# PKU-MARL/HARL

Hardware: AMD Instinct MI355X
Metric: transitions/sec through HAPPO update (MPE spread, 3 agents) (higher is better)
Workload: dtype f32; 1 GPU; MPE simple_spread_v2 3-agent HAPPO update: compute_returns + train(), T=200, n_rollout_threads=4096/GPU (4096 global, weak scaling), obs18/share54/Box5, MLP[128, 128], ppo_epoch=5, critic_epoch=5; episode_length=200, n_rollout_threads_per_gpu=4096, n_rollout_threads_global=4096, n_agents=3, parallelism=dp1, collective=none, world_size=1, ranks_seen=1

## Files before the change

### harl_amd/csrc/bwd_fused.h

```cpp
#pragma once

__device__ __forceinline__ unsigned split_stage1(float f0, float f1, float &r0, float &r1) {
  const unsigned b0 = __float_as_uint(f0), b1 = __float_as_uint(f1);
  r0 = f0 - __uint_as_float(b0 & 0xffff0000u);
  r1 = f1 - __uint_as_float(b1 & 0xffff0000u);
  return __builtin_amdgcn_perm(b1, b0, 0x07060302u);
}
__device__ __forceinline__ void split_stage2(float r0, float r1, unsigned &p2, unsigned &p3) {
  const unsigned c0 = __float_as_uint(r0), c1 = __float_as_uint(r1);
  p2 = __builtin_amdgcn_perm(c1, c0, 0x07060302u);
  const float q0 = r0 - __uint_as_float(c0 & 0xffff0000u), q1 = r1 - __uint_as_float(c1 & 0xffff0000u);
  p3 = __builtin_amdgcn_perm(__float_as_uint(q1), __float_as_uint(q0), 0x07060302u);
}

template <int I, int N, typename F>
__device__ __forceinline__ void static_for(F &&f) {
  if constexpr (I < N) {
    f(std::integral_constant<int, I>{});
    static_for<I + 1, N>(f);
  }
}

constexpr int BDW_H = 128, BDW_MT = 4, BDW_NJ = 8, BDW_NR = 64, BDW_KPF = 32;
constexpr int BDW_SQ = (128 / 16) * 128 + 8, BDW_IMG = 8 * BDW_SQ;
constexpr int BDW_BUF = 3 * BDW_IMG;
constexpr size_t bdw_lds_bytes() { return split_image_bytes(128, 128) + (size_t)2 * BDW_BUF; }

template <int N>
__device__ __forceinline__ void zero_acc(f32x16 (&a)[N], float *db = nullptr) {
#pragma unroll
  for (int t = 0; t < N; ++t) {
    if (db) db[t] = 0.f;
#pragma unroll
    for (int r = 0; r < 16; ++r) a[t][r] = 0.f;
  }
}

struct GradRounds {
  static constexpr int H = BDW_H;
  const float *const dz, *const xprev;
  const long n_slabs;
  unsigned char *const Bb;
  const int lane, wave, i, h;
  const Ident ident;
  f32x16 acc2[4];
  float db2;
  f32x4 prA[4], prB[4];
  u32x2_t spB[4][3];
  u32x4 ya[3][2];
  f32x16 tc[3];
  u32x4 At[3][2], AtN[3][2];
  float rr0, rr1;
  float vnext;
  const int frag_lane;

  __device__ __forceinline__ GradRounds(const float *dz_, const float *xprev_, long n_slabs_, unsigned char *Bb_, int lane_,
                                        int wave_, const Ident &ident_)
      : dz(dz_), xprev(xprev_), n_slabs(n_slabs_), Bb(Bb_), lane(lane_), wave(wave_), i(lane_ & 31), h(lane_ >> 5),
        ident(ident_), db2(0.f), rr0(0.f), rr1(0.f), vnext(1.f),
        frag_lane(((lane_ >> 4) & 1) * 128 + ((lane_ & 15) >> 2) * 32 + (lane_ & 3) * 8) {}

  __device__ __forceinline__ void d_load(long ds) {
#pragma unroll
    for (int u = 0; u < 4; ++u) {
      prA[u] = (reinterpret_cast<const f32x4 *>(dz + ds * (long)(H * SLAB)) + lane)[(4 * wave + u) * WAVE];
      prB[u] = (reinterpret_cast<const f32x4 *>(xprev + ds * (long)(H * SLAB)) + lane)[(4 * wave + u) * WAVE];
    }
  }
  __device__ __forceinline__ void d_load_next(long ds, long fallback) { d_load(ds < n_slabs ? ds : fallback); }
  __device__ __forceinline__ void a_chunk(int k) {
    const int pi = k >> 1, j = pi >> 2, c = pi & 3, u = pi >> 1, e = 2 * (pi & 1);
    if ((k & 1) == 0) {
      ya[0][j][c] = split_stage1(prA[u][e], prA[u][e + 1], rr0, rr1);
    } else {
      unsigned p2, p3;
      split_stage2(rr0, rr1, p2, p3);
      ya[1][j][c] = p2;
      ya[2][j][c] = p3;
    }
  }
  __device__ __forceinline__ void b_chunk(int k) {
    const int u = k >> 2, c2 = (k >> 1) & 1;
    if ((k & 1) == 0) {
      spB[u][0][c2] = split_stage1(prB[u][2 * c2], prB[u][2 * c2 + 1], rr0, rr1);
    } else {
      unsigned p2, p3;
      split_stage2(rr0, rr1, p2, p3);
      spB[u][1][c2] = p2;
      spB[u][2][c2] = p3;
    }
  }
  __device__ __forceinline__ void t_mfma(int k) {
    const f32x16 zero = {0.f, 0.f, 0.f, 0.f, 0.f, 0.f, 0.f, 0.f, 0.f, 0.f, 0.f, 0.f, 0.f, 0.f, 0.f, 0.f};
    const int t = k % 3;
    if (k < 3) tc[t] = mfma_bf16(ya[t][0], ident.j0, zero);
    else tc[t] = mfma_bf16(ya[t][1], ident.j1, tc[t]);
  }
  __device__ __forceinline__ void p_chunk(int k) {
    if (k < 3) {
      pack_transposed(tc[k], AtN[k][0], AtN[k][1]);
    } else {
      f32x2 a = {0.f, 0.f};
#pragma unroll
      for (int r = 0; r < 8; ++r) a += f32x2{tc[k - 3][2 * r], tc[k - 3][2 * r + 1]};
      db2 += vnext * (a[0] + a[1]);
    }
  }
  __device__ __forceinline__ void b_store(int buf) {
#pragma unroll
    for (int u = 0; u < 4; ++u) {
      const int q = 4 * wave + u;
      unsigned char *d = Bb + buf * BDW_BUF + (i >> 2) * BDW_SQ + (2 * (q >> 2) + ((q & 3) >> 1)) * 128 + (i & 3) * 32 +
                         (8 * (q & 1) + 4 * h) * 2;
#pragma unroll
      for (int term = 0; term < 3; ++term) *reinterpret_cast<u32x2_t *>(d + term * BDW_IMG) = spB[u][term];
    }
  }
  __device__ __forceinline__ void read_frag(int buf, int ks, int tile, u32x4 (&f)[3]) {
#pragma unroll
    for (int term = 0; term < 3; ++term) {
      const unsigned char *fp = Bb + buf * BDW_BUF + term * BDW_IMG + (4 * ks + h) * BDW_SQ + 2 * tile * 128 + frag_lane;
      const u32x2_t lo = tr_read(fp), hi = tr_read(fp + 2 * BDW_SQ);
      f[term] = u32x4{lo[0], lo[1], hi[0], hi[1]};
    }
  }
  __device__ __forceinline__ void a_advance() {
#pragma unroll
    for (int t = 0; t < 3; ++t) {
      At[t][0] = AtN[t][0];
      At[t][1] = AtN[t][1];
    }
  }

  __device__ __forceinline__ void prologue(long base0) {
    d_load(base0);
#pragma unroll
    for (int k = 0; k < 16; ++k) a_chunk(k);
#pragma unroll
    for (int k = 0; k < 6; ++k) t_mfma(k);
#pragma unroll
    for (int k = 0; k < 16; ++k) b_chunk(k);
#pragma unroll
    for (int k = 0; k < 6; ++k) p_chunk(k);
    a_advance();
    b_store(0);
  }

  template <int r, bool FILL, class Sched, class Extra, class Phase>
  __device__ __forceinline__ void round(long base, long sr_stride, Extra &&extra, Phase &&phase) {
    __syncthreads();
    phase(std::integral_constant<int, 5>{});
    const long ds1 = r < 3 ? base + r + 1 : base + sr_stride;
    const long ds2 = r < 2 ? base + r + 2 : base + sr_stride;
    vnext = uniform_f(ds1 < n_slabs ? 1.f : 0.f);
    constexpr int TSLOT = r == 0 ? 31 : 15;
    auto slot = [&](auto sc) {
      constexpr int s_ = decltype(sc)::value;
      if constexpr (r == 0) {
        if constexpr (s_ >= 16 && s_ < 32) a_chunk(s_ - 16);
        else if constexpr (s_ >= 32 && s_ < 42) b_chunk(s_ - 32 + 6);
        else if constexpr (s_ >= 42) p_chunk(s_ - 42);
        if constexpr (s_ == Sched::LOAD_R0) d_load_next(ds2, base);
      } else {
        if constexpr (s_ < 16) a_chunk(s_);
        else if constexpr (s_ < 26) b_chunk(s_ - 16 + 6);
        else if constexpr (s_ < 32) p_chunk(s_ - 26);
        else extra(std::integral_constant<int, r>{}, sc);
        if constexpr (s_ == Sched::LOAD_RN && r < 3) d_load_next(ds2, base);
      }
      if constexpr (s_ == TSLOT) {
        static_for<0, 6>([&](auto kc) {
          constexpr int k = decltype(kc)::value;
          __builtin_amdgcn_sched_barrier(0);
          t_mfma(k);
          b_chunk(k);
        });
      }
    };
    u32x4 bv[2][3];
    read_frag(r & 1, 0, 0, bv[0]);
    if constexpr (!FILL) static_for<0, 48>(slot);
    static_for<0, 8>([&](auto nc) {
      constexpr int n = decltype(nc)::value, ks = n >> 2, b = n & 3;
      if constexpr (n + 1 < 8) read_frag(r & 1, (n + 1) >> 2, (n + 1) & 3, bv[(n + 1) & 1]);
      __builtin_amdgcn_sched_barrier(0);
      constexpr int AT[6] = {2, 0, 1, 1, 0, 0}, BT[6] = {0, 2, 1, 0, 1, 0};
      static_for<0, 6>([&](auto kc) {
        constexpr int k6 = decltype(kc)::value;
        acc2[b] = mfma_bf16(At[AT[k6]][ks], bv[n & 1][BT[k6]], acc2[b]);
        if constexpr (FILL) slot(std::integral_constant<int, 6 * n + k6>{});
        __builtin_amdgcn_sched_barrier(0);
      });
    });
    phase(std::integral_constant<int, 6>{});
    b_store((r + 1) & 1);
    a_advance();
    phase(std::integral_constant<int, 7>{});
  }

  template <bool FILL, class Sched, class Extra, class Phase>
  __device__ __forceinline__ void rounds(long base, long sr_stride, Extra &&extra, Phase &&phase) {
    static_for<0, 4>([&](auto rc) {
      constexpr int r = decltype(rc)::value;
      if (base + r < n_slabs) round<r, FILL, Sched>(base, sr_stride, extra, phase);
    });
  }

  __device__ __forceinline__ void store_row(float *dw2_part) {
    float *mypart = dw2_part + (long)blockIdx.x * ((long)H * H + H);
#pragma unroll
    for (int b = 0; b < 4; ++b)
#pragma unroll
      for (int r = 0; r < 16; ++r) {
        const int o = 32 * wave + (r & 3) + 8 * (r >> 2) + 4 * h;
        mypart[(long)o * H + 32 * b + i] = acc2[b][r];
      }
    const float dbt = wave_sum32(db2);
    if (h == 0) mypart[(long)H * H + 32 * wave + i] = dbt;
  }
};

template <int NTH>
__device__ __forceinline__ void clear_dw2_rows(float *dw2_part, int n_part_rows) {
  constexpr long ROW2 = (long)BDW_H * BDW_H + BDW_H;
  for (int row = blockIdx.x + gridDim.x; row < n_part_rows; row += gridDim.x) {
    float *z = dw2_part + (long)row * ROW2;
    for (int e = threadIdx.x; e < ROW2; e += NTH) z[e] = 0.f;
  }
}

__device__ __forceinline__ void owner_split_chunk(int k, const float (&raw)[BDW_NR], u32x4 (&g1)[BDW_NJ], u32x4 (&g2)[BDW_NJ],
                                                  u32x4 (&g3)[BDW_NJ], float &q0, float &q1) {
  const int pi = k >> 1, j = pi >> 2, c = pi & 3;
  if ((k & 1) == 0) {
    g1[j][c] = split_stage1(raw[2 * pi], raw[2 * pi + 1], q0, q1);
  } else {
    unsigned p2, p3;
    split_stage2(q0, q1, p2, p3);
    g2[j][c] = p2;
    g3[j][c] = p3;
  }
}
__device__ __forceinline__ void owner_ln_operands(const float *xprev, const float *rstd_prev, const uint32_t *mask_prev, long slab,
                                                  int lane, float (&xh)[BDW_NR], float &rstd, uint32_t (&mbits)[2]) {
  atl_load<BDW_H>(xprev, slab, lane, xh);
  rstd = rstd_prev[slab * SLAB + (lane & 31)];
#pragma unroll
  for (int w = 0; w < 2; ++w) mbits[w] = mask_prev[(slab * 2 + w) * WAVE + lane];
}
__device__ __forceinline__ void owner_x0_operands(const float *x0n, long slab, int lane, f32x4 (&x0r)[BDW_KPF / 8]) {
  const f32x4 *bp = reinterpret_cast<const f32x4 *>(x0n + slab * (long)(BDW_KPF * SLAB)) + lane;
#pragma unroll
  for (int q = 0; q < BDW_KPF / 8; ++q) x0r[q] = bp[q * WAVE];
}
__device__ __forceinline__ void owner_ln_bwd(const f32x16 (&acc)[BDW_MT], const float (&xh)[BDW_NR], const uint32_t (&mbits)[2],
                                             float rstd, float *dz_prev, long slab, int lane, float (&out)[BDW_NR]) {
  float dx[BDW_NR];
#pragma unroll
  for (int R = 0; R < BDW_NR; ++R) dx[R] = acc[R >> 4][R & 15];
  ln_bwd_relu_mbits<BDW_H>(dx, xh, mbits, rstd, out);
  if (dz_prev) atl_store<BDW_H>(dz_prev, slab, lane, out);
}
struct Dw1Acc {
  f32x16 acc1[4];
  float dbs[4];
  __device__ __forceinline__ void zero() { zero_acc(acc1, dbs); }
  __device__ __forceinline__ void add(const f32x4 (&x0r)[BDW_KPF / 8], const float (&out)[BDW_NR], const Ident &ident) {
    float xr0[BDW_KPF / 2];
#pragma unroll
    for (int q = 0; q < BDW_KPF / 8; ++q)
#pragma unroll
      for (int e = 0; e < 4; ++e) xr0[4 * q + e] = x0r[q][e];
    u32x4 a1[BDW_KPF / 16], a2[BDW_KPF / 16], a3[BDW_KPF / 16];
    split_acts<BDW_KPF / 2>(xr0, a1, a2, a3);
    u32x4 Bt[3][2];
    transpose_block<false>(a1[0], a1[1], a2[0], a2[1], a3[0], a3[1], ident, Bt);
#pragma unroll
    for (int a = 0; a < 4; ++a) {
      u32x4 A1[3][2];
      dbs[a] += split_transpose_block<true>(&out[16 * a], ident, A1);
      dw_tile(acc1[a], A1, Bt);
    }
  }
  template <int NTH>
  __device__ __forceinline__ void finish(float *buf, float *dw1_part, int n_part_rows) {
    f32x16 a1x[4][1];
#pragma unroll
    for (int a = 0; a < 4; ++a) a1x[a][0] = acc1[a];
    finish_partials<4, 1, NTH>(a1x, dbs, buf, dw1_part, n_part_rows);
  }
};

struct Sched4 { static constexpr int LOAD_R0 = 41, LOAD_RN = 25; };
template <int KT, bool FILL>
__global__ __launch_bounds__(WG_THREADS, 1) void k_bwd_dx_dw(
    const float *__restrict__ dz, const float *__restrict__ xprev, const uint32_t *__restrict__ mask_prev,
    const float *__restrict__ rstd_prev, const float *__restrict__ Wp, float *__restrict__ dz_prev, long n_slabs,
    const float *__restrict__ x0n, float *__restrict__ dw1_part, float *__restrict__ dw2_part, int n_part_rows) {
  constexpr int H = BDW_H, MT = BDW_MT, NJ = BDW_NJ, NR = BDW_NR, KPF = BDW_KPF;
  extern __shared__ __attribute__((aligned(16))) float lds[];
  PHASE_BEGIN();
  auto ph = [&](auto pc) { PHASE(decltype(pc)::value); };
  u32x4 *img = reinterpret_cast<u32x4 *>(lds);
  stage_split_matrix<H, H, true, WG_THREADS>(img, Wp);
  __syncthreads();
  const int lane = threadIdx.x & 63, wave = wave_id();
  const u32x4 *wl = img + lane;
  const long sr_stride = (long)gridDim.x * WAVES_PER_WG;
  const long base0 = (long)blockIdx.x * WAVES_PER_WG;
  const Ident ident = make_ident(lane);

  GradRounds G(dz, xprev, n_slabs, reinterpret_cast<unsigned char *>(img + 3 * MT * NJ * 64), lane, wave, ident);
  Dw1Acc A1;
  zero_acc(G.acc2);
  if constexpr (KT > 0) A1.zero();

  float raw[NR];
  u32x4 g1[NJ], g2[NJ], g3[NJ];
  float ro0 = 0.f, ro1 = 0.f;
  auto o_chunk = [&](int k) { owner_split_chunk(k, raw, g1, g2, g3, ro0, ro1); };
  atl_load<H>(dz, base0 + wave < n_slabs ? base0 + wave : 0, lane, raw);
#pragma unroll
  for (int k = 0; k < 8; ++k) o_chunk(k);
  if (base0 < n_slabs) G.prologue(base0);
  PHASE(10);

  for (long base = base0; base < n_slabs; base += sr_stride) {
    const long slab = base + wave;
    const bool own = slab < n_slabs;
    const long nxt = slab + sr_stride < n_slabs ? slab + sr_stride : (own ? slab : 0);
    if (own) {
      float xh[NR], rstd;
      uint32_t mbits[2];
      owner_ln_operands(xprev, rstd_prev, mask_prev, slab, lane, xh, rstd, mbits);
      f32x4 x0r[KT > 0 ? KPF / 8 : 1];
      if constexpr (KT > 0) owner_x0_operands(x0n, slab, lane, x0r);
      f32x16 acc[MT];
      zero_acc(acc);
      PHASE(0);
      split_gemm_fill<MT, NJ>(wl, g1, g2, g3, acc, [&](int s_, int k6) {
        const int j1 = s_ / MT + 1, q = (s_ % MT) * 6 + k6;
        if (j1 < NJ && q % 3 == 0) o_chunk(8 * j1 + q / 3);
      });
      PHASE(1);
      float out[NR];
      owner_ln_bwd(acc, xh, mbits, rstd, dz_prev, slab, lane, out);
      PHASE(2);
      if constexpr (KT > 0) {
        A1.add(x0r, out, ident);
        PHASE(3);
      }
    }
    atl_load<H>(dz, nxt, lane, raw);
    G.d_load_next(base + 1, base);
    PHASE(4);
    G.rounds<FILL, Sched4>(base, sr_stride, [&](auto rc, auto sc) {
      constexpr int r = decltype(rc)::value, s_ = decltype(sc)::value;
      if constexpr (r == 3 && s_ < 40) o_chunk(s_ - 32);
    }, ph);
  }

  G.store_row(dw2_part);
  clear_dw2_rows<WG_THREADS>(dw2_part, n_part_rows);
  if constexpr (KT > 0) A1.finish<WG_THREADS>(reinterpret_cast<float *>(img), dw1_part, n_part_rows);
  PHASE(11);
  PHASE_END(3);
}

#ifndef HARL_BWD_SPLIT_WAVES
#define HARL_BWD_SPLIT_WAVES 1
#endif
struct Sched8 { static constexpr int LOAD_R0 = 47, LOAD_RN = 31; };
template <int KT, bool FILL>
__global__ __launch_bounds__(2 * WG_THREADS, 1) void k_bwd_dx_dw8(
    const float *__restrict__ dz, const float *__restrict__ xprev, const uint32_t *__restrict__ mask_prev,
    const float *__restrict__ rstd_prev, const float *__restrict__ Wp, float *__restrict__ dz_prev, long n_slabs,
    const float *__restrict__ x0n, float *__restrict__ dw1_part, float *__restrict__ dw2_part, int n_part_rows) {
  constexpr int H = BDW_H, MT = BDW_MT, NJ = BDW_NJ, NR = BDW_NR, KPF = BDW_KPF, NTH = 2 * WG_THREADS;
  extern __shared__ __attribute__((aligned(16))) float lds[];
  PHASE_BEGIN();
  auto ph = [&](auto pc) { PHASE(decltype(pc)::value); };
  u32x4 *img = reinterpret_cast<u32x4 *>(lds);
  stage_split_matrix<H, H, true, NTH>(img, Wp);
  __syncthreads();
  const int lane = threadIdx.x & 63, wave_ = wave_id();
  const int wave = wave_ & 3;
  const bool owner = wave_ < WAVES_PER_WG;
  const u32x4 *wl = img + lane;
  const long sr_stride = (long)gridDim.x * WAVES_PER_WG;
  const long base0 = (long)blockIdx.x * WAVES_PER_WG;
  const Ident ident = make_ident(lane);

  GradRounds G(dz, xprev, n_slabs, reinterpret_cast<unsigned char *>(img + 3 * MT * NJ * 64), lane, wave, ident);
  Dw1Acc A1;
// ... 90 lines not shown
```

### harl_amd/csrc/split_mfma.h

```cpp
#pragma once
#include "common.h"

typedef unsigned u32x4 __attribute__((ext_vector_type(4)));
typedef unsigned u32x2_t __attribute__((ext_vector_type(2)));
typedef __bf16 bf16x8 __attribute__((ext_vector_type(8)));

namespace harl {

__device__ __forceinline__ f32x16 mfma_bf16(const u32x4 &a, const u32x4 &b, const f32x16 &c) {
  return __builtin_amdgcn_mfma_f32_32x32x16_bf16(__builtin_bit_cast(bf16x8, a), __builtin_bit_cast(bf16x8, b), c, 0, 0, 0);
}

template <bool PACKED = PK_DEFAULT>
__device__ __forceinline__ void split3(float f0, float f1, unsigned &p1, unsigned &p2, unsigned &p3) {
  const unsigned b0 = __float_as_uint(f0), b1 = __float_as_uint(f1);
  p1 = __builtin_amdgcn_perm(b1, b0, 0x07060302u);
  if constexpr (PACKED) {
    const f32x2 r = f32x2{f0, f1} - f32x2{__uint_as_float(b0 & 0xffff0000u), __uint_as_float(b1 & 0xffff0000u)};
    const unsigned c0 = __float_as_uint(r[0]), c1 = __float_as_uint(r[1]);
    p2 = __builtin_amdgcn_perm(c1, c0, 0x07060302u);
    const f32x2 q = r - f32x2{__uint_as_float(c0 & 0xffff0000u), __uint_as_float(c1 & 0xffff0000u)};
    p3 = __builtin_amdgcn_perm(__float_as_uint(q[1]), __float_as_uint(q[0]), 0x07060302u);
  } else {
    const float r0 = f0 - __uint_as_float(b0 & 0xffff0000u), r1 = f1 - __uint_as_float(b1 & 0xffff0000u);
    const unsigned c0 = __float_as_uint(r0), c1 = __float_as_uint(r1);
    p2 = __builtin_amdgcn_perm(c1, c0, 0x07060302u);
    const float q0 = r0 - __uint_as_float(c0 & 0xffff0000u), q1 = r1 - __uint_as_float(c1 & 0xffff0000u);
    p3 = __builtin_amdgcn_perm(__float_as_uint(q1), __float_as_uint(q0), 0x07060302u);
  }
}

__device__ __forceinline__ unsigned cvt_pk_bf16(float lo, float hi) {
  unsigned r;
  asm("v_cvt_pk_bf16_f32 %0, %1, %2" : "=v"(r) : "v"(lo), "v"(hi));
  return r;
}
__device__ __forceinline__ void split3_rne(float f0, float f1, unsigned &p1, unsigned &p2, unsigned &p3) {
  p1 = cvt_pk_bf16(f0, f1);
  const float r0 = f0 - __uint_as_float(p1 << 16), r1 = f1 - __uint_as_float(p1 & 0xffff0000u);
  p2 = cvt_pk_bf16(r0, r1);
  const float q0 = r0 - __uint_as_float(p2 << 16), q1 = r1 - __uint_as_float(p2 & 0xffff0000u);
  p3 = cvt_pk_bf16(q0, q1);
}

template <int NR, bool PACKED = PK_DEFAULT>
__device__ __forceinline__ void split_acts(const float (&v)[NR], u32x4 (&x1)[NR / 8], u32x4 (&x2)[NR / 8], u32x4 (&x3)[NR / 8]) {
#pragma unroll
  for (int j = 0; j < NR / 8; ++j)
#pragma unroll
    for (int c = 0; c < 4; ++c) {
      unsigned a, b, d;
      split3<PACKED>(v[8 * j + 2 * c], v[8 * j + 2 * c + 1], a, b, d);
      x1[j][c] = a;
      x2[j][c] = b;
      x3[j][c] = d;
    }
}

constexpr size_t split_image_bytes(int rows, int k) { return (size_t)3 * rows * k * 2; }

void launch_split_image(const float *Wp, int H, int D, int KP, void *img, hipStream_t stream);

template <int HO, int HI, bool TRANSPOSED, int NTHR>
__device__ __forceinline__ void stage_split_matrix(u32x4 *__restrict__ img, const float *__restrict__ Wp) {
  constexpr int M = TRANSPOSED ? HI : HO, K = TRANSPOSED ? HO : HI, MT = M / 32, NJ = K / 16;
  constexpr int TOTAL = MT * NJ * 64, PER = (TOTAL + NTHR - 1) / NTHR;
  float w[PER][8];
#pragma unroll
  for (int u = 0; u < PER; ++u) {
    const int e = threadIdx.x + u * NTHR, ec = e < TOTAL ? e : 0;
    const int ln = ec & 63, j = (ec >> 6) % NJ, t = (ec >> 6) / NJ, m = 32 * t + (ln & 31), g = ln >> 5;
#pragma unroll
    for (int c = 0; c < 8; ++c) {
      const int k = feat_base(8 * j + c) + 4 * g;
      w[u][c] = TRANSPOSED ? Wp[(long)k * HI + m] : Wp[(long)m * HI + k];
    }
  }
#pragma unroll
  for (int u = 0; u < PER; ++u) {
    const int e = threadIdx.x + u * NTHR;
    if (e < TOTAL) {
      unsigned p[3][4];
#pragma unroll
      for (int c = 0; c < 4; ++c) split3_rne(w[u][2 * c], w[u][2 * c + 1], p[0][c], p[1][c], p[2][c]);
#pragma unroll
      for (int term = 0; term < 3; ++term) img[term * TOTAL + e] = u32x4{p[term][0], p[term][1], p[term][2], p[term][3]};
    }
  }
}

template <int MT, int NJ, typename PRE>
__device__ __forceinline__ void split_gemm(const u32x4 *__restrict__ wl, const u32x4 (&x1)[NJ], const u32x4 (&x2)[NJ],
                                           const u32x4 (&x3)[NJ], f32x16 (&acc)[MT], PRE &&pre) {
  constexpr int TS = MT * NJ * 64;
  u32x4 wb[2][3];
#pragma unroll
  for (int term = 0; term < 3; ++term) wb[0][term] = wl[term * TS];
#pragma unroll
  for (int s = 0; s < MT * NJ; ++s) {
    const int j = s / MT, t = s % MT, cur = s & 1, nxt = cur ^ 1;
    if (s + 1 < MT * NJ) {
      const int j1 = (s + 1) / MT, t1 = (s + 1) % MT;
#pragma unroll
      for (int term = 0; term < 3; ++term) wb[nxt][term] = wl[term * TS + (t1 * NJ + j1) * 64];
    }
    pre(s);
    __builtin_amdgcn_sched_barrier(0);
    acc[t] = mfma_bf16(wb[cur][2], x1[j], acc[t]);
    acc[t] = mfma_bf16(wb[cur][0], x3[j], acc[t]);
    acc[t] = mfma_bf16(wb[cur][1], x2[j], acc[t]);
    acc[t] = mfma_bf16(wb[cur][1], x1[j], acc[t]);
    acc[t] = mfma_bf16(wb[cur][0], x2[j], acc[t]);
    acc[t] = mfma_bf16(wb[cur][0], x1[j], acc[t]);
    __builtin_amdgcn_sched_barrier(0);
  }
}

template <int MT, int NJ, typename FILLF>
__device__ __forceinline__ void split_gemm_fill(const u32x4 *__restrict__ wl, const u32x4 (&x1)[NJ], const u32x4 (&x2)[NJ],
                                                const u32x4 (&x3)[NJ], f32x16 (&acc)[MT], FILLF &&fill) {
  constexpr int TS = MT * NJ * 64;
  u32x4 wb[2][3];
#pragma unroll
  for (int term = 0; term < 3; ++term) wb[0][term] = wl[term * TS];
#pragma unroll
  for (int s = 0; s < MT * NJ; ++s) {
    const int j = s / MT, t = s % MT, cur = s & 1, nxt = cur ^ 1;
    if (s + 1 < MT * NJ) {
      const int j1 = (s + 1) / MT, t1 = (s + 1) % MT;
#pragma unroll
      for (int term = 0; term < 3; ++term) wb[nxt][term] = wl[term * TS + (t1 * NJ + j1) * 64];
    }
    __builtin_amdgcn_sched_barrier(0);
    acc[t] = mfma_bf16(wb[cur][2], x1[j], acc[t]);
    fill(s, 0);
    __builtin_amdgcn_sched_barrier(0);
    acc[t] = mfma_bf16(wb[cur][0], x3[j], acc[t]);
    fill(s, 1);
    __builtin_amdgcn_sched_barrier(0);
    acc[t] = mfma_bf16(wb[cur][1], x2[j], acc[t]);
    fill(s, 2);
    __builtin_amdgcn_sched_barrier(0);
    acc[t] = mfma_bf16(wb[cur][1], x1[j], acc[t]);
    fill(s, 3);
    __builtin_amdgcn_sched_barrier(0);
    acc[t] = mfma_bf16(wb[cur][0], x2[j], acc[t]);
    fill(s, 4);
    __builtin_amdgcn_sched_barrier(0);
    acc[t] = mfma_bf16(wb[cur][0], x1[j], acc[t]);
    fill(s, 5);
    __builtin_amdgcn_sched_barrier(0);
  }
}

}
```

### harl_amd/csrc/update.hip

```cpp
#include <type_traits>
#include "common.h"
#include "split_mfma.h"
#include "heads_common.h"
#include "mfma_transpose.h"
#include "../../include/harl_hip.h"

using namespace harl;

namespace {

int bad(const char *m) {
  set_error(m);
  return -2;
}

template <int H, bool MASK>
__device__ __forceinline__ void relu_ln(const f32x16 (&acc)[H / 32], float (&v)[H / 2], uint32_t (&bits)[(H / 2 + 31) / 32],
                                        float &rstd_out) {
  constexpr int NR = H / 2;
#pragma unroll
  for (int w = 0; w < (NR + 31) / 32; ++w) bits[w] = 0u;
#pragma unroll
  for (int R = 0; R < NR; ++R) {
    if constexpr (MASK) v[R] = relu_push(acc[R >> 4][R & 15], bits[R >> 5]);
// ... 118 lines not shown
      split_gemm<MT, NJ1>(wl1, a1, a2, a3, acc, [](int) {});
      uint32_t bits[NW];
      float r1;
      relu_ln<H, false>(acc, x1, bits, r1);
#pragma unroll
      for (int b = 0; b < MT; ++b) {
        u32x4 B[3][2];
        split_transpose_block<false, false>(&x1[16 * b], I, B);
#pragma unroll
        for (int term = 0; term < 3; ++term)
#pragma unroll
          for (int ks = 0; ks < 2; ++ks) pk[((b * 3 + term) * 2 + ks) * 64] = B[term][ks];
      }
    }
    __builtin_amdgcn_sched_barrier(0);
    u32x4 A[MT][3][2];
#pragma unroll
    for (int a = 0; a < MT; ++a) dbs[a] += split_transpose_block<true, false>(&raw[16 * a], I, A[a]);
#pragma unroll
    for (int b = 0; b < MT; ++b) {
      u32x4 B[3][2];
#pragma unroll
      for (int term = 0; term < 3; ++term)
#pragma unroll
        for (int ks = 0; ks < 2; ++ks) B[term][ks] = pk[((b * 3 + term) * 2 + ks) * 64];
#pragma unroll
      for (int a = 0; a < MT; ++a) dw_tile(acc2[a][b], A[a], B);
    }
  }
  finish_partials<MT, MT>(acc2, dbs, reinterpret_cast<float *>(park), part, n_part_rows);
}

template <int H, int KP0>
__global__ __launch_bounds__(WG_THREADS, 1) void k_upd_dx(const float *__restrict__ x0n, const float *__restrict__ dz2,
                                                          const float *__restrict__ W1p, int D,
                                                          const float *__restrict__ b1p, const float *__restrict__ W2p,
                                                          long n_slabs, float *__restrict__ part, int n_part_rows) {
  extern __shared__ __attribute__((aligned(16))) float lds[];
  constexpr int MT = H / 32, KT = KP0 / 32, NJ1 = KP0 / 16, NJ2 = H / 16, NR = H / 2, NW = (NR + 31) / 32;
  u32x4 *img2 = reinterpret_cast<u32x4 *>(lds);
  u32x4 *w1img = img2 + 3 * MT * NJ2 * 64;
  float *b1l = reinterpret_cast<float *>(w1img + 3 * MT * NJ1 * 64);
  stage_split_matrix<H, H, true, WG_THREADS>(img2, W2p);
  stage_w1_images<H, KP0, WG_THREADS>(w1img, W1p, D);
  for (int e = threadIdx.x; e < H; e += WG_THREADS) b1l[e] = b1p[e];
  __syncthreads();
  const int lane = threadIdx.x & 63, wave = wave_id(), h = lane >> 5;
  const long slab0 = (long)blockIdx.x * WAVES_PER_WG + wave, slab_stride = (long)gridDim.x * WAVES_PER_WG;
  const u32x4 *wl1 = w1img + lane, *wl2 = img2 + lane;
  const Ident I = make_ident(lane);
  f32x16 acc1[MT][KT];
  float dbs[MT];
#pragma unroll
  for (int a = 0; a < MT; ++a) {
    dbs[a] = 0.f;
#pragma unroll
    for (int n = 0; n < KT; ++n)
#pragma unroll
      for (int r = 0; r < 16; ++r) acc1[a][n][r] = 0.f;
  }
  float raw[NR], xr[KP0 / 2];
  atl_load<H>(dz2, slab0 < n_slabs ? slab0 : 0, lane, raw);
  atl_load<KP0>(x0n, slab0 < n_slabs ? slab0 : 0, lane, xr);
  for (long slab = slab0; slab < n_slabs; slab += slab_stride) {
    u32x4 a1[NJ1], a2[NJ1], a3[NJ1];
    split_acts<KP0 / 2>(xr, a1, a2, a3);
    float dx[NR];
    {
      u32x4 g1[NJ2], g2[NJ2], g3[NJ2];
      split_acts<NR>(raw, g1, g2, g3);
      const long nxt = slab + slab_stride < n_slabs ? slab + slab_stride : slab;
      atl_load<H>(dz2, nxt, lane, raw);
      atl_load<KP0>(x0n, nxt, lane, xr);
      f32x16 acc[MT];
#pragma unroll
      for (int t = 0; t < MT; ++t)
#pragma unroll
        for (int r = 0; r < 16; ++r) acc[t][r] = 0.f;
      split_gemm<MT, NJ2>(wl2, g1, g2, g3, acc, [](int) {});
#pragma unroll
      for (int R = 0; R < NR; ++R) dx[R] = acc[R >> 4][R & 15];
    }
    float dz1[NR];
    {
      float x1[NR];
      uint32_t bits1[NW];
      float r1;
      f32x16 acc[MT];
#pragma unroll
      for (int t = 0; t < MT; ++t)
#pragma unroll
        for (int r = 0; r < 16; ++r) acc[t][r] = b1l[32 * t + (r & 3) + 8 * (r >> 2) + 4 * h];
      split_gemm<MT, NJ1>(wl1, a1, a2, a3, acc, [](int) {});
      relu_ln<H, true>(acc, x1, bits1, r1);
      ln_bwd_relu_bits<H>(dx, x1, bits1, r1, dz1);
    }
    u32x4 B[KT][3][2];
#pragma unroll
    for (int n = 0; n < KT; ++n)
      transpose_block<false>(a1[2 * n], a1[2 * n + 1], a2[2 * n], a2[2 * n + 1], a3[2 * n], a3[2 * n + 1], I, B[n]);
#pragma unroll
    for (int a = 0; a < MT; ++a) {
      u32x4 A[3][2];
      dbs[a] += split_transpose_block<true>(&dz1[16 * a], I, A);
#pragma unroll
      for (int n = 0; n < KT; ++n) dw_tile(acc1[a][n], A, B[n]);
    }
  }
  finish_partials<MT, KT>(acc1, dbs, reinterpret_cast<float *>(img2), part, n_part_rows);
}

struct UpdFwdArgs {
  const float *x0n, *W1p, *b1p, *W2p, *b2p;
  int D;
  long n_slabs;
  float *dz2;
  int n_part_rows;
  float *xh1;
  uint32_t *mask1;
  float *rstd1;
};

constexpr int UF_WAVES = 8, UF_THREADS = 64 * UF_WAVES;

template <int NV>
__device__ __forceinline__ void block_reduce_store8(float (&v)[NV], float *red , float *out_row) {
  const int lane = threadIdx.x & 63, wave = wave_id();
#pragma unroll
  for (int k = 0; k < NV; ++k) {
    float t = wave_reduce_sum(v[k]);
    if (lane == 0) red[wave * PS_STRIDE + k] = t;
  }
  __syncthreads();
  if (threadIdx.x < PS_STRIDE) {
    float t = 0.f;
    if (threadIdx.x < NV) {
#pragma unroll
      for (int w = 0; w < UF_WAVES; ++w) t += red[w * PS_STRIDE + threadIdx.x];
    }
    out_row[threadIdx.x] = t;
  }
}

template <int H, int KP0, int DA, bool DISCRETE, bool TRAIN, typename ARGS>
__global__ __launch_bounds__(UF_THREADS, 2) void k_upd_fwd(UpdFwdArgs U, ARGS A) {
  constexpr bool CRITIC = std::is_same<ARGS, CriticArgs>::value;
  static_assert(DA >= 1 && DA <= 8 && (!CRITIC || DA == 1), "the LDS head-gradient tile covers 8 head outputs");
  constexpr int DAP = DA <= 4 ? 4 : 8;
  constexpr int HROWS = DA;
  constexpr bool HID = KP0 == 0;
  constexpr bool EARLY_X0N = H == 128 && KP0 == 32 && DA <= 5 && !DISCRETE;
  constexpr bool EARLY_X0N_LP = !TRAIN && !HID && (H == 64 || (DA != 4 && !(KP0 == 64 && DA >= 7 && !DISCRETE)));
  static_assert(!HID || TRAIN, "the last-layer variant exists for optimiser steps only");
  extern __shared__ __attribute__((aligned(16))) float lds[];
  PHASE_BEGIN();
  constexpr int MT = H / 32, NJ1 = KP0 / 16, NJ2 = H / 16, NR = H / 2, NW = (NR + 31) / 32;
  u32x4 *w2img = reinterpret_cast<u32x4 *>(lds);
  u32x4 *w1img = w2img + 3 * MT * NJ2 * 64;
  float *b1l = reinterpret_cast<float *>(w1img + 3 * MT * NJ1 * 64);
  float *b2l = b1l + H;
  float *whlT = b2l + H;
  float *cst = whlT + 2 * head_t_block(H, DA);
  float *red = cst + 7 * DAP;
  float *hacc = red + UF_WAVES * PS_STRIDE;
  const int lane = threadIdx.x & 63, wave = wave_id(), i = lane & 31, h = lane >> 5;
  const long slab0 = (long)wave * gridDim.x + blockIdx.x, slab_stride = (long)gridDim.x * UF_WAVES;
  constexpr int NXR = HID ? NR : KP0 / 2;
  float xr[NXR];
  atl_load<2 * NXR>(U.x0n, slab0 < U.n_slabs ? slab0 : 0, lane, xr);
  constexpr bool ROWS = !CRITIC || TRAIN;
  long rawn = 0;
  if constexpr (ROWS) rawn = row_index_request(A.idx, A.Whp, slab0, lane, A.M);
  stage_split_matrix<H, H, false, UF_THREADS>(w2img, U.W2p);
  if constexpr (!HID) stage_w1_images<H, KP0, UF_THREADS>(w1img, U.W1p, U.D);
  for (int e = threadIdx.x; e < H; e += UF_THREADS) {
    if constexpr (!HID) b1l[e] = U.b1p[e];
    b2l[e] = U.b2p[e];
  }
  if (TRAIN)
    for (int e = threadIdx.x; e < UF_WAVES * HROWS * H; e += UF_THREADS) hacc[e] = 0.f;
  if (threadIdx.x < WG_THREADS) {
    stage_head_t<H, DAP, DA>(whlT, cst, A.Whp, A.bhp, WG_THREADS);
    if constexpr (!CRITIC) {
      if (!DISCRETE) {
        for (int e = threadIdx.x; e < DAP; e += WG_THREADS) {
          float sg = 0.5f, sig = 1.f, lsig = 0.f, dsd = 0.f;
          if (e < A.act_dim) {
            sg = 1.0f / (1.0f + expf(-A.log_std[e] / A.std_x_coef));
            sig = sg * A.std_y_coef;
            lsig = logf(sig);
            dsd = A.std_y_coef * sg * (1.f - sg) / A.std_x_coef;
          }
          cst[DAP + e] = sig;
          cst[2 * DAP + e] = lsig;
          cst[3 * DAP + e] = dsd;
          cst[5 * DAP + e] = 1.0f / sig;
          cst[6 * DAP + e] = 1.0f / (sig * sig);
        }
      }
    }
  }
  __syncthreads();

  const u32x4 *wl1 = w1img + lane, *wl2 = w2img + lane;
  const float *whlT_h = whlT + h * head_t_block(H, DA);
  float *hw = hacc + wave * (HROWS * H);

  float adv_mean = 0.f, adv_den = 1.f, vmean = 0.f, vsd = 1.f;
  if constexpr (CRITIC) {
    if (TRAIN && A.vn_stats) {
      const float d = fmaxf(A.vn_stats[2], 1e-5f);
      vmean = A.vn_stats[0] / d;
      const float msq = A.vn_stats[1] / d;
      vsd = sqrtf(fmaxf(msq - vmean * vmean, 1e-2f));
    }
  } else {
    if (TRAIN && A.adv_moments) {
      const double cnt = A.adv_moments[2];
      const double m = A.adv_moments[0] / cnt;
      const double var = A.adv_moments[1] / cnt - m * m;
      adv_mean = (float)m;
      adv_den = 1.0f / ((float)sqrt(var > 0 ? var : 0.0) + 1e-5f);
    }
  }
  adv_mean = uniform_f(adv_mean);
  adv_den = uniform_f(adv_den);
  vmean = uniform_f(vmean);
  vsd = uniform_f(vsd);
  constexpr int NSC = CRITIC ? 8 : 8 + DAP;
  float sc[NSC];
#pragma unroll
  for (int k = 0; k < NSC; ++k) sc[k] = 0.f;
  float dbacc[CRITIC ? DAP : 1];
#pragma unroll
  for (int d = 0; d < (CRITIC ? DAP : 1); ++d) dbacc[d] = 0.f;

  __builtin_amdgcn_s_waitcnt(0x0F70);
  PHASE(10);
  for (long slab = slab0; slab < U.n_slabs; slab += slab_stride) {
    ActorRow<DAP> rcur;
    float cvold = 0.f, cret = 0.f;
    if constexpr (ROWS) {
      const long row = row_index_resolve(A.idx, rawn, slab, lane, A.M);
      if constexpr (!CRITIC) actor_row_load_at<DAP, DISCRETE, TRAIN, DA>(A, slab, lane, row, rcur);
      else critic_row_load_at(A, row, cvold, cret);
      rawn = row_index_request(A.idx, A.Whp, slab + slab_stride, lane, A.M);
      __builtin_amdgcn_sched_barrier(0);
    }
    float v[NR];
    uint32_t bits2[NW];
    float r2;
    {
      float x1[NR];
      if constexpr (HID) {
#pragma unroll
        for (int R = 0; R < NR; ++R) x1[R] = xr[R];
        PHASE(0);
        PHASE(1);
      } else {
        u32x4 a1[NJ1], a2[NJ1], a3[NJ1];
        split_acts<KP0 / 2>(xr, a1, a2, a3);
        if constexpr (EARLY_X0N_LP) atl_load<2 * NXR>(U.x0n, slab + slab_stride < U.n_slabs ? slab + slab_stride : slab, lane, xr);
        f32x16 acc[MT];
#pragma unroll
        for (int t = 0; t < MT; ++t)
#pragma unroll
          for (int r = 0; r < 16; ++r) acc[t][r] = b1l[32 * t + (r & 3) + 8 * (r >> 2) + 4 * h];
        PHASE(0);
        split_gemm<MT, NJ1>(wl1, a1, a2, a3, acc, [](int) {});
        PHASE(1);
        uint32_t bits1[NW];
        float r1;
        relu_ln<H, TRAIN>(acc, x1, bits1, r1);
        if constexpr (TRAIN) {
          if (U.xh1) {
            atl_store<H>(U.xh1, slab, lane, x1);
#pragma unroll
            for (int w = 0; w < NW; ++w) U.mask1[(slab * NW + w) * WAVE + lane] = bits1[w];
            if (lane < 32) U.rstd1[slab * SLAB + lane] = r1;
          }
        }
      }
      u32x4 y1[NJ2], y2[NJ2], y3[NJ2];
      split_acts<NR>(x1, y1, y2, y3);
      PHASE(2);
      f32x16 acc[MT];
#pragma unroll
      for (int t = 0; t < MT; ++t)
#pragma unroll
        for (int r = 0; r < 16; ++r) acc[t][r] = b2l[32 * t + (r & 3) + 8 * (r >> 2) + 4 * h];
      split_gemm<MT, NJ2>(wl2, y1, y2, y3, acc, [](int) {});
      PHASE(3);
      relu_ln<H, TRAIN>(acc, v, bits2, r2);
    }
    PHASE(4);
    f32x4 xs[H / 8];
#pragma unroll
    for (int q = 0; q < H / 8; ++q) xs[q] = f32x4{v[4 * q], v[4 * q + 1], v[4 * q + 2], v[4 * q + 3]};
    float z[DAP];
    head_fwd_regs_t<H, DAP, DA>(xs, whlT_h, cst, z);
    PHASE(5);
    const long sn = slab + slab_stride < U.n_slabs ? slab + slab_stride : slab;
    if constexpr (!TRAIN && !EARLY_X0N_LP) atl_load<2 * NXR>(U.x0n, sn, lane, xr);
    float dzh[DAP];
    float s1, s2;
    if constexpr (CRITIC) {
      float dv;
      if (!critic_sample<TRAIN>(A, z[0], slab, lane, vmean, vsd, sc, dv, cvold, cret)) continue;
#pragma unroll
      for (int d = 0; d < DAP; ++d) dzh[d] = d == 0 ? dv : 0.f;
      s1 = dv * cst[4 * DAP];
      s2 = dv * (z[0] - cst[0]);
    } else {
      if (!actor_sample<DAP, DISCRETE, TRAIN, DA>(A, cst, z, slab, lane, adv_mean, adv_den, sc, dzh, s1, s2, rcur)) continue;
    }
    PHASE(6);
    if constexpr (TRAIN) {
      if constexpr (EARLY_X0N) atl_load<2 * NXR>(U.x0n, sn, lane, xr);
      int lane_o = lane;
      asm volatile("" : "+v"(lane_o));
      const Ident I = make_ident(lane_o);
      const u32x4 I16 = make_ident16(lane_o);
      u32x4 Ah[3][2];
      {
        float e8[8];
#pragma unroll
        for (int c = 0; c < 8; ++c) e8[c] = (c < DAP && h == 0) ? dzh[c < DAP ? c : 0] : 0.f;
        u32x4 t1, t2, t3;
#pragma unroll
        for (int c = 0; c < 4; ++c) {
          unsigned a, b, d;
          split3(e8[2 * c], e8[2 * c + 1], a, b, d);
          t1[c] = a;
          t2[c] = b;
          t3[c] = d;
        }
        const f32x16 zero = {0.f, 0.f, 0.f, 0.f, 0.f, 0.f, 0.f, 0.f, 0.f, 0.f, 0.f, 0.f, 0.f, 0.f, 0.f, 0.f};
        const f32x16 c1 = mfma_bf16(t1, I16, zero), c2 = mfma_bf16(t2, I16, zero), c3 = mfma_bf16(t3, I16, zero);
        pack_transposed(c1, Ah[0][0], Ah[0][1]);
        pack_transposed(c2, Ah[1][0], Ah[1][1]);
        pack_transposed(c3, Ah[2][0], Ah[2][1]);
      }
#pragma unroll
      for (int n = 0; n < MT; ++n) {
        u32x4 B[3][2];
        split_transpose_block<false>(&v[16 * n], I, B);
        f32x16 tile = {0.f, 0.f, 0.f, 0.f, 0.f, 0.f, 0.f, 0.f, 0.f, 0.f, 0.f, 0.f, 0.f, 0.f, 0.f, 0.f};
        dw_tile(tile, Ah, B);
#pragma unroll
        for (int r = 0; r < 4; ++r) {
          if (r < HROWS && h == 0) hw[r * H + 32 * n + i] += tile[r];
          if (4 + r < HROWS && h == 1) hw[(4 + r) * H + 32 * n + i] += tile[r];
        }
      }
      if constexpr (CRITIC) {
        if (h == 0) dbacc[0] += dzh[0];
      } else {
        if (h == 1) {
#pragma unroll
          for (int d = 0; d < DAP; ++d) sc[8 + d] += dzh[d];
        }
      }
      PHASE(7);
      if constexpr (!EARLY_X0N) atl_load<2 * NXR>(U.x0n, sn, lane, xr);
      head_bwd_regs_bits<H, DAP, DA, true, true>(xs, bits2[0], bits2[NW - 1], r2, slab, lane, whlT, dzh, s1, s2, U.dz2);
      PHASE(8);
    }
  }
  if constexpr (TRAIN) {
    float dbv[DAP];
#pragma unroll
    for (int d = 0; d < DAP; ++d) {
      if constexpr (CRITIC) {
        dbv[d] = dbacc[d];
      } else {
        dbv[d] = h == 1 ? sc[8 + d] : 0.f;
        sc[8 + d] = h == 0 ? sc[8 + d] : 0.f;
      }
    }
    block_reduce_store8<NSC>(sc, red, A.part_scalars + (long)blockIdx.x * PS_STRIDE);
    for (int row = blockIdx.x + gridDim.x; row < U.n_part_rows; row += gridDim.x)
      if (threadIdx.x < PS_STRIDE) A.part_scalars[(long)row * PS_STRIDE + threadIdx.x] = 0.f;
    float dbs[DAP];
#pragma unroll
    for (int d = 0; d < DAP; ++d) dbs[d] = wave_reduce_sum(dbv[d]);
    float *dbl = red;
    __syncthreads();
    if (lane == 0) {
#pragma unroll
      for (int d = 0; d < DAP; ++d) dbl[wave * PS_STRIDE + d] = dbs[d];
    }
    __syncthreads();
    float *out = A.dw_part + (long)blockIdx.x * HeadDw<H>::OUT_FLOATS;
    for (int e = threadIdx.x; e < HeadDw<H>::OUT_FLOATS; e += UF_THREADS) {
      float t = 0.f;
      if (e < 32 * H) {
        const int row = e / H;
        if (row < HROWS) {
#pragma unroll
          for (int w = 0; w < UF_WAVES; ++w) t += hacc[(w * HROWS + row) * H + (e - row * H)];
        }
      } else {
        const int d = e - 32 * H;
        if (d < DAP) {
#pragma unroll
          for (int w = 0; w < UF_WAVES; ++w) t += dbl[w * PS_STRIDE + d];
        }
      }
      out[e] = t;
    }
    for (int row = blockIdx.x + gridDim.x; row < U.n_part_rows; row += gridDim.x) {
      float *zr = A.dw_part + (long)row * HeadDw<H>::OUT_FLOATS;
      for (int e = threadIdx.x; e < HeadDw<H>::OUT_FLOATS; e += UF_THREADS) zr[e] = 0.f;
    }
  }
  PHASE(11);
  PHASE_END((TRAIN ? 0 : 2) + (CRITIC ? 1 : 0));
}

int fwd_grid(long n_slabs) {
  const long wgs = (n_slabs + UF_WAVES - 1) / UF_WAVES;
  return (int)(wgs < 256 ? (wgs < 1 ? 1 : wgs) : 256);
}

int upd_grid(long n_slabs) {
  const long wgs = (n_slabs + WAVES_PER_WG - 1) / WAVES_PER_WG;
  return (int)(wgs < 256 ? (wgs < 1 ? 1 : wgs) : 256);
}

size_t fwd_lds_bytes(int H, int kp0, int dap, int hrows, int da) {
  return split_image_bytes(H, H) + split_image_bytes(H, kp0) +
         ((size_t)2 * H + (size_t)2 * head_t_block(H, da) + 7 * dap + UF_WAVES * PS_STRIDE + (size_t)UF_WAVES * hrows * H) *
             sizeof(float);
}

constexpr size_t LDS_PER_WG_MAX = 160 * 1024;

template <int H, int KP0, int DA, bool DISC, bool TRAIN, typename ARGS>
int launch_fwd(const UpdFwdArgs &U, const ARGS &A, hipStream_t s) {
  const size_t shm = fwd_lds_bytes(H, KP0, DA <= 4 ? 4 : 8, TRAIN ? DA : 0, DA);
  if (shm > LDS_PER_WG_MAX) {
    return bad("harl_update_*: this (D, H, act_dim) does not fit the LDS of one workgroup");
  }
  allow_big_lds(k_upd_fwd<H, KP0, DA, DISC, TRAIN, ARGS>, shm);
  hipLaunchKernelGGL((k_upd_fwd<H, KP0, DA, DISC, TRAIN, ARGS>), dim3(fwd_grid(U.n_slabs)), dim3(UF_THREADS), shm, s, U, A);
  return 0;
}

template <int H, int KP0, bool TRAIN, int DA = 8>
int launch_actor_width(const UpdFwdArgs &U, const ActorArgs &A, int discrete, hipStream_t s) {
  if (A.act_dim == DA)
    return discrete ? launch_fwd<H, KP0, DA, true, TRAIN, ActorArgs>(U, A, s) : launch_fwd<H, KP0, DA, false, TRAIN, ActorArgs>(U, A, s);
  if constexpr (DA > 1) return launch_actor_width<H, KP0, TRAIN, DA - 1>(U, A, discrete, s);
  return bad("harl_update_*: act_dim must be in [1, 8]");
}

template <bool TRAIN>
int dispatch_fwd_actor(const UpdFwdArgs &U, const ActorArgs &A, int H, int discrete, hipStream_t s) {
  const int D = A.act_dim;
  if (D < 1 || D > 8) return bad("harl_update_fwd: act_dim must be in [1, 8]");
  const int kp0 = U.D <= 32 ? 32 : 64;
#define CASE(Hv, Kv)                                                                \
  if (H == Hv && kp0 == Kv) {                                                       \
    const int rc = launch_actor_width<Hv, Kv, TRAIN>(U, A, discrete, s);             \
    return rc ? rc : check_launch("harl_update_fwd");                               \
  }
  CASE(128, 32) CASE(128, 64) CASE(64, 32) CASE(64, 64)
#undef CASE
  return bad("harl_update_fwd: hidden width must be 64 or 128");
}

int dispatch_last_actor(const UpdFwdArgs &U, const ActorArgs &A, int H, int discrete, hipStream_t s) {
  const int D = A.act_dim;
  if (D < 1 || D > 8) return bad("harl_update_last_actor: act_dim must be in [1, 8]");
  int rc;
  if (H == 128) rc = launch_actor_width<128, 0, true>(U, A, discrete, s);
  else if (H == 64) rc = launch_actor_width<64, 0, true>(U, A, discrete, s);
  else return bad("harl_update_last_actor: hidden width must be 64 or 128");
  return rc ? rc : check_launch("harl_update_last_actor");
}

int dispatch_last_critic(const UpdFwdArgs &U, const CriticArgs &A, int H, hipStream_t s) {
  int rc;
  if (H == 128) rc = launch_fwd<128, 0, 1, false, true, CriticArgs>(U, A, s);
  else if (H == 64) rc = launch_fwd<64, 0, 1, false, true, CriticArgs>(U, A, s);
  else return bad("harl_update_last_critic: hidden width must be 64 or 128");
  return rc ? rc : check_launch("harl_update_last_critic");
}

template <bool TRAIN>
int dispatch_fwd_critic(const UpdFwdArgs &U, const CriticArgs &A, int H, hipStream_t s) {
  const int kp0 = U.D <= 32 ? 32 : 64;
#define CASE(Hv, Kv)                                                     \
  if (H == Hv && kp0 == Kv) {                                            \
    const int rc = launch_fwd<Hv, Kv, 1, false, TRAIN, CriticArgs>(U, A, s); \
    return rc ? rc : check_launch("harl_update_fwd");                        \
  }
  CASE(128, 32) CASE(128, 64) CASE(64, 32) CASE(64, 64)
#undef CASE
  return bad("harl_update_fwd: hidden width must be 64 or 128");
}

}

HARL_PHASE_ACCESSOR(update)

extern "C" int harl_update_supported(int D, int H, int act_dim, int kind) {
  if (!(D >= 0 && D <= 64 && (H == 64 || H == 128) && act_dim >= 1 && act_dim <= 8)) return 0;
  const int dap = act_dim <= 4 ? 4 : 8;
  const int hrows = kind == 0 ? 0 : (kind == 2 ? 1 : act_dim);
  return fwd_lds_bytes(H, D == 0 ? 0 : (D <= 32 ? 32 : 64), dap, hrows, kind == 2 ? 1 : act_dim) <= LDS_PER_WG_MAX ? 1 : 0;
}

extern "C" int harl_update_fwd_actor(const float *x0n, long M, int D, int H, const float *W1p, const float *b1p,
                                     const float *W2p, const float *b2p, const float *Whp, const float *bhp,
                                     const float *log_std, float std_x_coef, float std_y_coef, int discrete, int act_dim,
                                     const float *actions, const float *avail, const float *old_logp, const float *adv,
                                     const double *adv_moments, const float *factor, const float *active,
                                     double clip_param, float entropy_coef, int agg_mean, int trpo, float *logp_out,
                                     float *dz2, float *part_scalars, float *dw_part_head, int n_part_rows, float *xh1,
                                     uint32_t *rmask1, float *rstd1, void *stream) {
// ... 142 lines not shown
```

Baseline: 54.09 million transitions/s.

## Interleave activation bf16 splitting into layer-2 MFMA stream and alternate wave priority

Instead of splitting all layer-1 activations into three bf16 parts before the layer-2 split GEMM, only the first chunk is split up front. The remaining chunks are split inside the GEMM's fill callback, so the VALU split work is hidden between MFMA issues. It also alternates s_setprio across waves per slab iteration so paired waves take turns having issue priority. The aim is to overlap VALU and matrix work, at the cost of more register pressure and scheduling sensitivity.

```diff
diff --git a/harl_amd/csrc/bwd_fused.h b/harl_amd/csrc/bwd_fused.h
--- a/harl_amd/csrc/bwd_fused.h
+++ b/harl_amd/csrc/bwd_fused.h
@@ -1,17 +1,4 @@
 #pragma once
-
-__device__ __forceinline__ unsigned split_stage1(float f0, float f1, float &r0, float &r1) {
-  const unsigned b0 = __float_as_uint(f0), b1 = __float_as_uint(f1);
-  r0 = f0 - __uint_as_float(b0 & 0xffff0000u);
-  r1 = f1 - __uint_as_float(b1 & 0xffff0000u);
-  return __builtin_amdgcn_perm(b1, b0, 0x07060302u);
-}
-__device__ __forceinline__ void split_stage2(float r0, float r1, unsigned &p2, unsigned &p3) {
-  const unsigned c0 = __float_as_uint(r0), c1 = __float_as_uint(r1);
-  p2 = __builtin_amdgcn_perm(c1, c0, 0x07060302u);
-  const float q0 = r0 - __uint_as_float(c0 & 0xffff0000u), q1 = r1 - __uint_as_float(c1 & 0xffff0000u);
-  p3 = __builtin_amdgcn_perm(__float_as_uint(q1), __float_as_uint(q0), 0x07060302u);
-}
 
 template <int I, int N, typename F>
 __device__ __forceinline__ void static_for(F &&f) {
@@ -231,15 +218,7 @@
 
 __device__ __forceinline__ void owner_split_chunk(int k, const float (&raw)[BDW_NR], u32x4 (&g1)[BDW_NJ], u32x4 (&g2)[BDW_NJ],
                                                   u32x4 (&g3)[BDW_NJ], float &q0, float &q1) {
-  const int pi = k >> 1, j = pi >> 2, c = pi & 3;
-  if ((k & 1) == 0) {
-    g1[j][c] = split_stage1(raw[2 * pi], raw[2 * pi + 1], q0, q1);
-  } else {
-    unsigned p2, p3;
-    split_stage2(q0, q1, p2, p3);
-    g2[j][c] = p2;
-    g3[j][c] = p3;
-  }
+  split_acts_chunk<BDW_NR>(k, raw, g1, g2, g3, q0, q1);
 }
 __device__ __forceinline__ void owner_ln_operands(const float *xprev, const float *rstd_prev, const uint32_t *mask_prev, long slab,
                                                   int lane, float (&xh)[BDW_NR], float &rstd, uint32_t (&mbits)[2]) {
diff --git a/harl_amd/csrc/split_mfma.h b/harl_amd/csrc/split_mfma.h
--- a/harl_amd/csrc/split_mfma.h
+++ b/harl_amd/csrc/split_mfma.h
@@ -55,6 +55,32 @@
       x2[j][c] = b;
       x3[j][c] = d;
     }
+}
+
+__device__ __forceinline__ unsigned split_stage1(float f0, float f1, float &r0, float &r1) {
+  const unsigned b0 = __float_as_uint(f0), b1 = __float_as_uint(f1);
+  r0 = f0 - __uint_as_float(b0 & 0xffff0000u);
+  r1 = f1 - __uint_as_float(b1 & 0xffff0000u);
+  return __builtin_amdgcn_perm(b1, b0, 0x07060302u);
+}
+__device__ __forceinline__ void split_stage2(float r0, float r1, unsigned &p2, unsigned &p3) {
+  const unsigned c0 = __float_as_uint(r0), c1 = __float_as_uint(r1);
+  p2 = __builtin_amdgcn_perm(c1, c0, 0x07060302u);
+  const float q0 = r0 - __uint_as_float(c0 & 0xffff0000u), q1 = r1 - __uint_as_float(c1 & 0xffff0000u);
+  p3 = __builtin_amdgcn_perm(__float_as_uint(q1), __float_as_uint(q0), 0x07060302u);
+}
+template <int NR>
+__device__ __forceinline__ void split_acts_chunk(int k, const float (&v)[NR], u32x4 (&x1)[NR / 8], u32x4 (&x2)[NR / 8],
+                                                 u32x4 (&x3)[NR / 8], float &q0, float &q1) {
+  const int pi = k >> 1, j = pi >> 2, c = pi & 3;
+  if ((k & 1) == 0) {
+    x1[j][c] = split_stage1(v[2 * pi], v[2 * pi + 1], q0, q1);
+  } else {
+    unsigned p2, p3;
+    split_stage2(q0, q1, p2, p3);
+    x2[j][c] = p2;
+    x3[j][c] = p3;
+  }
 }
 
 constexpr size_t split_image_bytes(int rows, int k) { return (size_t)3 * rows * k * 2; }
diff --git a/harl_amd/csrc/update.hip b/harl_amd/csrc/update.hip
--- a/harl_amd/csrc/update.hip
+++ b/harl_amd/csrc/update.hip
@@ -294,6 +294,10 @@
   constexpr bool EARLY_X0N = H == 128 && KP0 == 32 && DA <= 5 && !DISCRETE;
   constexpr bool EARLY_X0N_LP = !TRAIN && !HID && (H == 64 || (DA != 4 && !(KP0 == 64 && DA >= 7 && !DISCRETE)));
   static_assert(!HID || TRAIN, "the last-layer variant exists for optimiser steps only");
+#ifndef HARL_UPD_RIDE_SPLIT
+#define HARL_UPD_RIDE_SPLIT 1
+#endif
+  constexpr bool RIDE_SPLIT = HARL_UPD_RIDE_SPLIT && TRAIN && H == 128 && !HID && !DISCRETE && !(KP0 == 32 && DA == 1 && !CRITIC);
   extern __shared__ __attribute__((aligned(16))) float lds[];
   PHASE_BEGIN();
   constexpr int MT = H / 32, NJ1 = KP0 / 16, NJ2 = H / 16, NR = H / 2, NW = (NR + 31) / 32;
@@ -379,7 +383,17 @@
 
   __builtin_amdgcn_s_waitcnt(0x0F70);
   PHASE(10);
+#ifndef HARL_UPD_PRIO
+#define HARL_UPD_PRIO 1
+#endif
+  constexpr bool PRIO = HARL_UPD_PRIO && RIDE_SPLIT;
+  int trip = wave >> 2;
   for (long slab = slab0; slab < U.n_slabs; slab += slab_stride) {
+    if constexpr (PRIO) {
+      if (trip & 1) __builtin_amdgcn_s_setprio(1);
+      else __builtin_amdgcn_s_setprio(0);
+      ++trip;
+    }
     ActorRow<DAP> rcur;
     float cvold = 0.f, cret = 0.f;
     if constexpr (ROWS) {
@@ -424,14 +438,27 @@
         }
       }
       u32x4 y1[NJ2], y2[NJ2], y3[NJ2];
-      split_acts<NR>(x1, y1, y2, y3);
+      float sq0 = 0.f, sq1 = 0.f;
+      if constexpr (RIDE_SPLIT) {
+#pragma unroll
+        for (int k = 0; k < 8; ++k) split_acts_chunk<NR>(k, x1, y1, y2, y3, sq0, sq1);
+      } else {
+        split_acts<NR>(x1, y1, y2, y3);
+      }
       PHASE(2);
       f32x16 acc[MT];
 #pragma unroll
       for (int t = 0; t < MT; ++t)
 #pragma unroll
         for (int r = 0; r < 16; ++r) acc[t][r] = b2l[32 * t + (r & 3) + 8 * (r >> 2) + 4 * h];
-      split_gemm<MT, NJ2>(wl2, y1, y2, y3, acc, [](int) {});
+      if constexpr (RIDE_SPLIT) {
+        split_gemm_fill<MT, NJ2>(wl2, y1, y2, y3, acc, [&](int s_, int k6) {
+          const int j1 = s_ / MT + 1, q = (s_ % MT) * 6 + k6;
+          if (j1 < NJ2 && q % 3 == 0) split_acts_chunk<NR>(8 * j1 + q / 3, x1, y1, y2, y3, sq0, sq1);
+        });
+      } else {
+        split_gemm<MT, NJ2>(wl2, y1, y2, y3, acc, [](int) {});
+      }
       PHASE(3);
       relu_ln<H, TRAIN>(acc, v, bits2, r2);
     }
@@ -509,6 +536,7 @@
       PHASE(8);
     }
   }
+  if constexpr (PRIO) __builtin_amdgcn_s_setprio(0);
   if constexpr (TRAIN) {
     float dbv[DAP];
 #pragma unroll
```

Measured after the change: 54.37 million transitions/s (median of 4 runs). About the same (+0.5%).
